# tbennun/capital

Hardware: NVIDIA H100
Metric: cholesky_tflops_fp64 (higher is better)
Workload: dtype f64

## Files before the change

capital_b200/csrc/api.cu:

```cuda
#include "common.cuh"
#include "dist.cuh"
#include "peer.cuh"
#include <math.h>
#include <stdlib.h>
#include <algorithm>

capital_status_t capital_ctx::workspace(const std::string& name, size_t bytes, void** out) {
  capital_ctx* ctx = this;
  DeviceBuf& b = pool[name];
  if (b.bytes < bytes) {
    if (b.p) CAP_CUDA(cudaFree(b.p));
    b.p = nullptr; b.bytes = 0;
    CAP_CUDA(cudaMalloc(&b.p, bytes));
    b.bytes = bytes;
    if (poison_workspace) {
      CAP_CUDA(cudaMemsetAsync(b.p, 0xFF, bytes, cudaStreamLegacy));
      CAP_CUDA(cudaStreamSynchronize(cudaStreamLegacy));
    }
  }
  *out = b.p;
  return CAPITAL_OK;
}

int capital_ctx::stream_id(cudaStream_t st) const {
  if (st == hi) return 1;
  if (st == side) return 2;
  if (st == side_deep[0]) return 3;
  if (st == side_deep[1]) return 4;
  if (peer) {
    const Peer* P = (const Peer*)peer;
    for (int q = 0; q < PEER_Q; q++) if (st == P->push[q]) return 5 + q;
  }
  if (st == copy_in) return 10;
  if (st == copy_out) return 11;
  return 0;
}
int capital_ctx::tl_begin(cudaStream_t st, int kind, double a, double b, double c) {
  if (!timeline) return -1;
  while (tl_pool.size() < tl_used + 2) {
    cudaEvent_t e;
    if (cudaEventCreate(&e) != cudaSuccess) return -1;
    tl_pool.push_back(e);
  }
  TlRec r{tl_pool[tl_used], tl_pool[tl_used + 1], stream_id(st), kind, a, b, c};
  tl_used += 2;
  cudaEventRecord(r.e0, st);
  tl.push_back(r);
  return (int)tl.size() - 1;
}
void capital_ctx::tl_end(cudaStream_t st, int idx) {
  if (idx >= 0) cudaEventRecord(tl[idx].e1, st);
}

bool cap_is_device_ptr(const void* p) {
  cudaPointerAttributes at;
  if (cudaPointerGetAttributes(&at, p) != cudaSuccess) { cudaGetLastError(); return false; }
  return at.type == cudaMemoryTypeDevice || at.type == cudaMemoryTypeManaged;
}

capital_status_t cap_stage_in(capital_ctx* ctx, const double* src, size_t count, const char* name, const double** out) {
  if (cap_is_device_ptr(src)) { *out = src; return CAPITAL_OK; }
  void* d;
  CAP_TRY(ctx->workspace(name, count * 8, &d));
  CAP_CUDA(cudaMemcpyAsync(d, src, count * 8, cudaMemcpyHostToDevice, ctx->stream));
  ctx->counters.h2d_bytes += (int64_t)count * 8;
  *out = (const double*)d;
  return CAPITAL_OK;
}
capital_status_t cap_stage_out_begin(capital_ctx* ctx, double* dst, size_t count, const char* name, double** dev) {
  if (cap_is_device_ptr(dst)) { *dev = dst; return CAPITAL_OK; }
  void* d;
  CAP_TRY(ctx->workspace(name, count * 8, &d));
  *dev = (double*)d;
  return CAPITAL_OK;
}
capital_status_t cap_stage_out_end(capital_ctx* ctx, double* dst, size_t count, const double* dev) {
  if (dev == dst) return CAPITAL_OK;
  CAP_CUDA(cudaMemcpyAsync(dst, dev, count * 8, cudaMemcpyDeviceToHost, ctx->stream));
  ctx->counters.d2h_bytes += (int64_t)count * 8;
  return CAPITAL_OK;
}

capital_status_t cap_check_info(capital_ctx* ctx) {
  int info = 0;
  CAP_CUDA(cudaMemcpyAsync(&info, ctx->d_info, sizeof(int), cudaMemcpyDeviceToHost, ctx->stream));
  CAP_CUDA(cudaStreamSynchronize(ctx->stream));
  if (info == -3) {
    ctx->set_error("the experimental TF32 trailing-update kernel gave up on an mbarrier wait (gemm_tf32.cu watchdog): results are invalid");
    return CAPITAL_ERR_CUDA;
  }
  if (info < 0) {
    ctx->set_error("a wait on a peer GPU timed out (a rank of the grid died, or the ranks did not make the same sequence of calls)");
    return CAPITAL_ERR_COMM;
  }
  if (info != 0) {
    ctx->set_error("matrix is not positive definite: non-positive pivot " + std::to_string(info) + " in a base-case block");
    return CAPITAL_ERR_NOT_SPD;
  }
  return CAPITAL_OK;
}

namespace {
struct HostIO {
  capital_ctx* ctx = nullptr;
  int64_t L = 0, ld = 0;
  double *Rm = nullptr, *Ri = nullptr, *dR = nullptr, *dRinv = nullptr, *hR = nullptr, *hRinv = nullptr;
  bool packed = true;
  std::vector<std::pair<int64_t, cudaEvent_t>> chunks;
  int64_t waited = 0;
  int64_t cols_out = 0, rinv_cols_out = 0;
  bool rinv_streams = false;
  cudaEvent_t e_out = nullptr;
};
capital_status_t io_event(capital_ctx* ctx, cudaEvent_t* e) {
  if (ctx->io_used == ctx->io_pool.size()) {
    cudaEvent_t ev;
    CAP_CUDA(cudaEventCreateWithFlags(&ev, cudaEventDisableTiming));
    ctx->io_pool.push_back(ev);
  }
  *e = ctx->io_pool[ctx->io_used++];
  return CAPITAL_OK;
}
capital_status_t hostio_need_cols(void* user, cudaStream_t st, int64_t col_end) {
  HostIO* io = (HostIO*)user;
  capital_ctx* ctx = io->ctx;
  if (col_end <= io->waited) return CAPITAL_OK;
  for (auto& ch : io->chunks)
    if (ch.first >= col_end) {
      CAP_CUDA(cudaStreamWaitEvent(st, ch.second, 0));
      io->waited = ch.first;
      return CAPITAL_OK;
    }
  return CAPITAL_OK;
}
capital_status_t hostio_left_done(void* user, cudaStream_t st, int64_t col_end, int depth) {
  HostIO* io = (HostIO*)user;
  capital_ctx* ctx = io->ctx;
  const int64_t c0 = io->cols_out;
  if (col_end <= c0) return CAPITAL_OK;
  const bool rinv_too = depth == 0 || (depth == 1 && io->rinv_streams && io->rinv_cols_out == c0);
  const size_t off = (size_t)c0 * (c0 + 1) / 2, cnt = (size_t)col_end * (col_end + 1) / 2 - off;
  cudaStream_t ps = (!ctx->no_overlap && !io->hR && !io->hRinv) ? ctx->copy_out : st;
  cudaEvent_t e;
  if (ps != st) {
    CAP_TRY(io_event(ctx, &e));
    CAP_CUDA(cudaEventRecord(e, st));
    CAP_CUDA(cudaStreamWaitEvent(ps, e, 0));
  }
  CAP_TRY(pack_upper(ctx, ps, io->L, io->Rm, io->ld, io->dR, 0, c0, col_end));
  if (rinv_too) CAP_TRY(pack_upper(ctx, ps, io->L, io->Ri, io->ld, io->dRinv, 0, c0, col_end));
  io->cols_out = col_end;
  if (rinv_too) io->rinv_cols_out = col_end;
  if (!io->hR && !io->hRinv) {
    if (ps != st) {
      CAP_TRY(io_event(ctx, &io->e_out));
      CAP_CUDA(cudaEventRecord(io->e_out, ps));
    }
    return CAPITAL_OK;
  }
  CAP_TRY(io_event(ctx, &e));
  CAP_CUDA(cudaEventRecord(e, ps));
  CAP_CUDA(cudaStreamWaitEvent(ctx->copy_out, e, 0));
  if (io->hR) { CAP_CUDA(cudaMemcpyAsync(io->hR + off, io->dR + off, cnt * 8, cudaMemcpyDeviceToHost, ctx->copy_out)); ctx->counters.d2h_bytes += (int64_t)cnt * 8; }
  if (io->hRinv && rinv_too) { CAP_CUDA(cudaMemcpyAsync(io->hRinv + off, io->dRinv + off, cnt * 8, cudaMemcpyDeviceToHost, ctx->copy_out)); ctx->counters.d2h_bytes += (int64_t)cnt * 8; }
  CAP_TRY(io_event(ctx, &io->e_out));
  CAP_CUDA(cudaEventRecord(io->e_out, ctx->copy_out));
  return CAPITAL_OK;
}
int64_t hostio_cols_waited(void* user) { return ((HostIO*)user)->waited; }
capital_status_t hostio_emit(HostIO* io, cudaStream_t st, bool r_part, int64_t col_end) {
  capital_ctx* ctx = io->ctx;
// ... 458 lines not shown
  const int64_t s1 = L >> args->split;
  const bool packed = structure == CAPITAL_UPPERTRI_PACKED;
  const size_t f_count = packed ? (size_t)L * (L + 1) / 2 : (size_t)L * L;
  const int64_t ldu = packed ? 0 : L;
  cudaStream_t st = ctx->stream;
  const double *dRi = nullptr, *dR = nullptr, *dB;
  if (!apply_r) CAP_TRY(cap_stage_in(ctx, Rinv_local, f_count, "solve_Rinv", &dRi));
  if (skipped || apply_r) CAP_TRY(cap_stage_in(ctx, R_local, f_count, "solve_R", &dR));
  CAP_TRY(cap_stage_in(ctx, B, (size_t)ldb * (nrhs - 1) + n, "solve_B", &dB));
  const bool x_host = !cap_is_device_ptr(X);
  double* dX = X;
  if (x_host) CAP_TRY(ctx->workspace("solve_X", (size_t)ldx * nrhs * 8, (void**)&dX));
  double *T, *T2;
  CAP_TRY(ctx->workspace("solve_T", (size_t)L * SOLVE_W * 8, (void**)&T));
  CAP_TRY(ctx->workspace("solve_T2", (size_t)L * SOLVE_W * 8, (void**)&T2));
  auto half_t = [&](const double* Bp, int64_t w) -> capital_status_t {
    if (!skipped) return tri_apply(ctx, st, {dRi, ldu, true, 0, L, 0, L, w, 1.0, Bp, 1, ldb, 0.0, nullptr, 0, T, 1, L});
    CAP_TRY(tri_apply(ctx, st, {dRi, ldu, true, 0, s1, 0, s1, w, 1.0, Bp, 1, ldb, 0.0, nullptr, 0, T, 1, L}));
    CAP_TRY(tri_apply(ctx, st, {dR, ldu, true, 0, s1, s1, L, w, -1.0, T, 1, L, 1.0, Bp, ldb, T2, 1, L}));
    return tri_apply(ctx, st, {dRi, ldu, true, s1, L, s1, L, w, 1.0, T2, 1, L, 0.0, nullptr, 0, T, 1, L});
  };
  auto half_n = [&](double* Xp, int64_t w) -> capital_status_t {
    if (!skipped) return tri_apply(ctx, st, {dRi, ldu, false, 0, L, 0, L, w, 1.0, T, 1, L, 0.0, nullptr, 0, Xp, 1, ldx});
    CAP_TRY(tri_apply(ctx, st, {dRi, ldu, false, s1, L, s1, L, w, 1.0, T, 1, L, 0.0, nullptr, 0, Xp, 1, ldx}));
    CAP_TRY(tri_apply(ctx, st, {dR, ldu, false, 0, s1, s1, L, w, -1.0, Xp, 1, ldx, 1.0, T, L, T2, 1, L}));
    return tri_apply(ctx, st, {dRi, ldu, false, 0, s1, 0, s1, w, 1.0, T2, 1, L, 0.0, nullptr, 0, Xp, 1, ldx});
  };
  for (int64_t p0 = 0; p0 < nrhs; p0 += SOLVE_W) {
    const int64_t w = std::min<int64_t>(SOLVE_W, nrhs - p0);
    const double* Bp = dB + p0 * ldb;
    double* Xp = dX + p0 * ldx;
    if (apply_r) {
      CAP_TRY(panel_add(ctx, st, L, w, Bp, ldb, nullptr, 0, T, L));
      CAP_TRY(tri_apply(ctx, st, {dR, ldu, mode == SOLVE_RT, 0, L, 0, L, w, 1.0, T, 1, L, 0.0, nullptr, 0, Xp, 1, ldx}));
      continue;
    }
    if (mode != SOLVE_RINV) CAP_TRY(half_t(Bp, w));
    else CAP_TRY(panel_add(ctx, st, L, w, Bp, ldb, nullptr, 0, T, L));
    if (mode != SOLVE_RINVT) CAP_TRY(half_n(Xp, w));
    else CAP_TRY(panel_add(ctx, st, L, w, T, L, nullptr, 0, Xp, ldx));
  }
  if (x_host) {
    CAP_CUDA(cudaMemcpy2DAsync(X, (size_t)ldx * 8, dX, (size_t)ldx * 8, (size_t)n * 8, (size_t)nrhs, cudaMemcpyDeviceToHost, st));
    ctx->counters.d2h_bytes += n * nrhs * 8;
    CAP_CUDA(cudaStreamSynchronize(st));
  }
  return CAPITAL_OK;
}

capital_status_t capital_cholinv_solve_f64(capital_ctx* ctx, int64_t n, const capital_cholinv_args_t* args, capital_structure_t structure,
                                           const double* R_local, const double* Rinv_local, int64_t nrhs, const double* B, int64_t ldb,
                                           double* X, int64_t ldx) {
  if (!ctx) return CAPITAL_ERR_INVALID;
  return cholinv_solve_mode(ctx, n, args, structure, R_local, Rinv_local, nrhs, B, ldb, X, ldx, SOLVE_FULL, "solve");
}

capital_status_t capital_cholinv_apply_rinv_f64(capital_ctx* ctx, int64_t n, const capital_cholinv_args_t* args, capital_structure_t structure,
                                                const double* R_local, const double* Rinv_local, int trans, int64_t nrhs, const double* B,
                                                int64_t ldb, double* X, int64_t ldx) {
  if (!ctx) return CAPITAL_ERR_INVALID;
  if (trans != 0 && trans != 1) {
    ctx->set_error("cholinv::apply_rinv: trans must be 0 (X = R^-1 B) or 1 (X = R^-T B)");
    return CAPITAL_ERR_INVALID;
  }
  return cholinv_solve_mode(ctx, n, args, structure, R_local, Rinv_local, nrhs, B, ldb, X, ldx, trans ? SOLVE_RINVT : SOLVE_RINV,
                            "apply_rinv");
}

capital_status_t capital_cholinv_apply_r_f64(capital_ctx* ctx, int64_t n, const capital_cholinv_args_t* args, capital_structure_t structure,
                                             const double* R_local, int trans, int64_t nrhs, const double* B, int64_t ldb, double* X,
                                             int64_t ldx) {
  if (!ctx) return CAPITAL_ERR_INVALID;
  if (trans != 0 && trans != 1) {
    ctx->set_error("cholinv::apply_r: trans must be 0 (X = R B) or 1 (X = R^T B)");
    return CAPITAL_ERR_INVALID;
  }
  return cholinv_solve_mode(ctx, n, args, structure, R_local, nullptr, nrhs, B, ldb, X, ldx, trans ? SOLVE_RT : SOLVE_R, "apply_r");
}

constexpr size_t BATCHED_WORKSPACE_CAP = size_t(2) << 30;

static int batched_cluster_width(int64_t nb) {
  const char* e = getenv("CAPITAL_BATCHED_CW");
  if (e && atoi(e) == 8) return 8;
  const int64_t T = nb / 64;
  return T <= 2 ? 2 : T <= 4 ? 4 : 8;
}

static bool all_device(std::initializer_list<const void*> ptrs) {
  for (const void* p : ptrs)
    if (!cap_is_device_ptr(p)) return false;
  return true;
}

capital_status_t capital_cholinv_factor_batched_f64(capital_ctx* ctx, int64_t n, int64_t batch, const double* A, double* R, double* Rinv,
                                                    int* info) {
  if (!ctx) return CAPITAL_ERR_INVALID;
  if (!A || !R || !Rinv || !info || n < 1 || batch < 1) {
    ctx->set_error("cholinv::factor_batched: invalid arguments (A, R, Rinv, info non-null, n >= 1, batch >= 1)");
    return CAPITAL_ERR_INVALID;
  }
  if (n > BASECASE_MAX) {
    ctx->set_error("cholinv::factor_batched: n > 512 is not supported (factor each matrix with capital_cholinv_factor_f64)");
    return CAPITAL_ERR_UNSUPPORTED;
  }
  CAP_CUDA(cudaSetDevice(ctx->device));
  if (!all_device({A, R, Rinv, info})) {
    ctx->set_error("cholinv::factor_batched: A, R, Rinv and info must be device pointers");
    return CAPITAL_ERR_INVALID;
  }
  cudaStream_t st = ctx->stream;
  const int64_t nn = n * n;
  CAP_CUDA(cudaMemsetAsync(info, 0, (size_t)batch * sizeof(int), st));
  if (n <= LEAF_MAX) {
    for (int64_t b0 = 0; b0 < batch; b0 += INT32_MAX) {
      const LeafBatch bt{std::min<int64_t>(INT32_MAX, batch - b0), {nn, nn, nn, 0}, info + b0, 0};
      CAP_TRY(leaf_cholinv(ctx, st, (int)n, A + b0 * nn, n, R + b0 * nn, n, Rinv + b0 * nn, n, nullptr, 0, &bt));
    }
    return CAPITAL_OK;
  }
  const int64_t nb = round_up(n, 64), mm = nb * nb;
  const bool direct = nb == n && (((uintptr_t)R | (uintptr_t)Rinv) & 15) == 0;
  const int64_t chunk = std::min<int64_t>({batch, 65535, (int64_t)(BATCHED_WORKSPACE_CAP / ((direct ? 2 : 4) * mm * 8))});
  double *W, *RiT, *Rw = nullptr, *Riw = nullptr;
  CAP_TRY(ctx->workspace("batched_W", (size_t)(chunk * mm) * 8, (void**)&W));
  CAP_TRY(ctx->workspace("batched_RiT", (size_t)(chunk * mm) * 8, (void**)&RiT));
  if (!direct) {
    CAP_TRY(ctx->workspace("batched_R", (size_t)(chunk * mm) * 8, (void**)&Rw));
    CAP_TRY(ctx->workspace("batched_Ri", (size_t)(chunk * mm) * 8, (void**)&Riw));
  }
  const int cw = batched_cluster_width(nb);
  for (int64_t b0 = 0; b0 < batch; b0 += chunk) {
    const int64_t cnt = std::min(chunk, batch - b0);
    CAP_TRY(sym_pad_batched(ctx, st, n, nb, cnt, A + b0 * nn, W));
    if (direct) {
      CAP_CUDA(cudaMemsetAsync(Rinv + b0 * nn, 0, (size_t)(cnt * nn) * 8, st));
      const LeafBatch bt{cnt, {mm, nn, nn, mm}, info + b0, cw};
      CAP_TRY(basecase_cholinv(ctx, st, (int)nb, W, nb, R + b0 * nn, n, Rinv + b0 * nn, n, RiT, nb, &bt));
    } else {
      const LeafBatch bt{cnt, {mm, mm, mm, mm}, info + b0, cw};
      CAP_TRY(basecase_cholinv(ctx, st, (int)nb, W, nb, Rw, nb, Riw, nb, RiT, nb, &bt));
      CAP_TRY(triu_out_batched(ctx, st, n, cnt, Rw, nb, mm, R + b0 * nn));
      CAP_TRY(triu_out_batched(ctx, st, n, cnt, Riw, nb, mm, Rinv + b0 * nn));
    }
  }
  return CAPITAL_OK;
}

capital_status_t capital_cholinv_solve_batched_f64(capital_ctx* ctx, int64_t n, int64_t batch, const double* Rinv, int64_t nrhs,
                                                   const double* B, double* X) {
  if (!ctx) return CAPITAL_ERR_INVALID;
  if (!Rinv || !B || !X || n < 1 || batch < 1 || nrhs < 1) {
    ctx->set_error("cholinv::solve_batched: invalid arguments (Rinv, B, X non-null, n >= 1, batch >= 1, nrhs >= 1)");
    return CAPITAL_ERR_INVALID;
  }
  if (n > BASECASE_MAX) {
    ctx->set_error("cholinv::solve_batched: n > 512 is not supported");
    return CAPITAL_ERR_UNSUPPORTED;
  }
  CAP_CUDA(cudaSetDevice(ctx->device));
  if (!all_device({Rinv, B, X})) {
    ctx->set_error("cholinv::solve_batched: Rinv, B and X must be device pointers");
    return CAPITAL_ERR_INVALID;
  }
  cudaStream_t st = ctx->stream;
  const int64_t nn = n * n, nbk = n * nrhs, ts = n * SOLVE_W;
  const int64_t per = (ts + round_up(n, 64) * SOLVE_W) * 8;
// ... 343 lines not shown
```

capital_b200/csrc/leaf.cu:

```cuda
#include "common.cuh"
#include <cooperative_groups.h>
#include <cfloat>
#include <stdlib.h>
#include <type_traits>
namespace cg = cooperative_groups;

namespace {
constexpr int LD = LEAF_MAX + 1;
constexpr int TLD = 68;
constexpr int TILE_DOUBLES = 64 * TLD;

__device__ __forceinline__ double fast_rsqrt(double d) {
  if (!(d > 1e-30 && d < 1e30)) return rsqrt(d);
  double y = (double)rsqrtf((float)d);
  const double h = 0.5 * d;
  y = y * fma(-h, y * y, 1.5);
  y = y * fma(-h, y * y, 1.5);
  return y;
}

__device__ void leaf_factor_invert(int nb, double* __restrict__ a, double* __restrict__ r, double* __restrict__ t, int* info,
                                   int pivot_base) {
  const int tid = threadIdx.x, tx = tid & 15, ty = tid >> 4;
  for (int k = 0; k < nb; k++) {
    if (tid < 64 && tid >= k && tid < nb) {
      double d = a[k + k * LD];
      if (!(d > 0.0)) {
        if (tid == k) atomicCAS(info, 0, pivot_base + k + 1);
        d = 1.0;
      }
      const double rs = rsqrt(d);
      r[k + tid * LD] = (tid == k) ? d * rs : a[k + tid * LD] * rs;
    }
    __syncthreads();
#pragma unroll
    for (int ia = 0; ia < 4; ia++) {
      const int i = ty + 16 * ia;
      if (i > k && i < nb) {
        const double ri = r[k + i * LD];
#pragma unroll
        for (int jb = 0; jb < 4; jb++) {
          const int j = tx + 16 * jb;
          if (j >= i && j < nb) a[i + j * LD] -= ri * r[k + j * LD];
        }
      }
    }
    __syncthreads();
  }
#pragma unroll
  for (int ia = 0; ia < 4; ia++) {
    const int i = ty + 16 * ia;
#pragma unroll
    for (int jb = 0; jb < 4; jb++) {
      const int j = tx + 16 * jb;
      if (i < nb && j < nb) {
        if (i > j) r[i + j * LD] = 0.0;
        a[i + j * LD] = (i == j) ? 1.0 / r[i + i * LD] : 0.0;
      }
    }
  }
  __syncthreads();
  int lg = 0;
  for (int bs = 1; bs < nb; bs <<= 1, lg++) {
    const int span = 2 * bs;
    const int npairs = (nb + span - 1) / span;
    const int per = bs * bs, total = npairs * per;
    for (int idx = tid; idx < total; idx += 256) {
      const int p = idx >> (2 * lg), e = idx & (per - 1);
      const int li = e & (bs - 1), lj = e >> lg;
      const int o = p * span, i = o + li, j = o + bs + lj;
      if (j < nb) {
        double s = 0.0;
        const int kend = o + bs;
        for (int k = i; k < kend; k++) s += a[i + k * LD] * r[k + j * LD];
        t[i + j * LD] = s;
      }
    }
    __syncthreads();
    for (int idx = tid; idx < total; idx += 256) {
      const int p = idx >> (2 * lg), e = idx & (per - 1);
      const int li = e & (bs - 1), lj = e >> lg;
      const int o = p * span, i = o + li, j = o + bs + lj;
      if (j < nb) {
        double s = 0.0;
        for (int k = o + bs; k <= j; k++) s += t[i + k * LD] * a[k + j * LD];
        a[i + j * LD] = -s;
      }
// ... 233 lines not shown
      sXb[(16 + jl) * TLD + i] = -s;
      sXTb[i * TLD + 16 + jl] = -s;
    });
    (void)tr;
  }
  __syncwarp();
  if (dbg2 && lane == 0) dbg2[2] = clock64();
}

__device__ __forceinline__ void mma32(double (&acc)[2][2], const double* As, int ar, const double* Bs, int bc, int k0) {
  const int lane = threadIdx.x & 31, w = threadIdx.x >> 5, g = lane >> 2, q = lane & 3;
  const double* ap = As + (ar + (w & 3) * 8 + g) * TLD + k0 + q;
  const double* bp = Bs + (bc + (w >> 2) * 16 + g) * TLD + k0 + q;
#pragma unroll
  for (int k = 0; k < 32; k += 4) {
    const double a = ap[k], b0 = bp[k], b1 = bp[8 * TLD + k];
    dmma884(acc[0][0], acc[0][1], a, b0);
    dmma884(acc[1][0], acc[1][1], a, b1);
  }
}
#define M32_ROW ((w & 3) * 8 + g)
#define M32_COL(j, e) ((w >> 2) * 16 + (j) * 8 + 2 * q + (e))

__device__ void leaf64_fast(double* __restrict__ sA, double* __restrict__ sR, double* __restrict__ sX, double* __restrict__ sXT,
                            double* __restrict__ ub, int* info, int pivot_base, long long* dbg2 = nullptr) {
  const int tid = threadIdx.x, lane = tid & 31, w = tid >> 5, g = lane >> 2, q = lane & 3;
  for (int idx = tid; idx < 64 * 64; idx += 256) {
    const int r = idx & 63, cidx = idx >> 6;
    sR[cidx * TLD + r] = 0.0; sX[cidx * TLD + r] = 0.0; sXT[cidx * TLD + r] = 0.0;
  }
  __syncthreads();
  double c[32];
#pragma unroll 1
  for (int half = 0; half < 2; half++) {
    const int o = half * 32;
    if (half == 1) {
      double acc[2][2] = {{0.0, 0.0}, {0.0, 0.0}};
      mma32(acc, sX, 0, sA, 32, 0);
#pragma unroll
      for (int j = 0; j < 2; j++)
#pragma unroll
        for (int e = 0; e < 2; e++) sR[(32 + M32_COL(j, e)) * TLD + M32_ROW] = acc[j][e];
      __syncthreads();
      double acc2[2][2] = {{0.0, 0.0}, {0.0, 0.0}};
      mma32(acc2, sR + 32 * TLD, 0, sR + 32 * TLD, 0, 0);
#pragma unroll
      for (int j = 0; j < 2; j++)
#pragma unroll
        for (int e = 0; e < 2; e++) sA[(32 + M32_COL(j, e)) * TLD + 32 + M32_ROW] -= acc2[j][e];
      __syncthreads();
    }
    if (w == 0) {
#pragma unroll
      for (int i = 0; i < 32; i++) c[i] = sA[(o + lane) * TLD + o + i];
      warp_potrf_trtri_32(c, sR + o * TLD + o, sX + o * TLD + o, sXT + o * TLD + o, ub, lane, info, pivot_base + o,
                          (dbg2 && half == 0) ? dbg2 : nullptr);
      if (dbg2 && half == 0 && lane == 0) dbg2[3] = clock64();
    }
    __syncthreads();
  }
  {
    double acc[2][2] = {{0.0, 0.0}, {0.0, 0.0}};
    mma32(acc, sXT, 0, sR, 32, 0);
    __syncthreads();
#pragma unroll
    for (int j = 0; j < 2; j++)
#pragma unroll
      for (int e = 0; e < 2; e++) sA[M32_ROW * TLD + 32 + M32_COL(j, e)] = acc[j][e];
    __syncthreads();
    double acc2[2][2] = {{0.0, 0.0}, {0.0, 0.0}};
    mma32(acc2, sA, 0, sX, 32, 32);
#pragma unroll
    for (int j = 0; j < 2; j++)
#pragma unroll
      for (int e = 0; e < 2; e++) {
        const double v = -acc2[j][e];
        sX[(32 + M32_COL(j, e)) * TLD + M32_ROW] = v;
        sXT[M32_ROW * TLD + 32 + M32_COL(j, e)] = v;
      }
  }
  __syncthreads();
}

template <int CW>
__global__ void __cluster_dims__(CW, 1, 1) __launch_bounds__(256, 1)
    basecase_kernel(int nb, double* __restrict__ W, long long ldw, double* __restrict__ R, long long ldr, double* __restrict__ Ri,
                    long long ldri, double* __restrict__ RiT, long long ldrit, int* __restrict__ info, long long* __restrict__ dbg,
                    BatchStrides bstr) {
  {
    const long long b = blockIdx.y;
    W += b * bstr.w; R += b * bstr.r; Ri += b * bstr.ri; RiT += b * bstr.rit; info += b;
  }
  extern __shared__ __align__(16) double sm[];
  double* sA = sm;
  double* sB = sm + TILE_DOUBLES;
  double* sT = sm + 2 * TILE_DOUBLES;
  cg::cluster_group cluster = cg::this_cluster();
  const int rank = (int)cluster.block_rank();
  const int T = nb >> 6;
  double acc[4][2][2];
  int dbgi = 0;
#define DBG_STAMP() do { if (dbg && rank == 0 && threadIdx.x == 0) dbg[dbgi++] = clock64(); } while (0)
  DBG_STAMP();

  double* sU = sm + 3 * TILE_DOUBLES;
  auto do_leaf = [&](int jb) {
    const long long o = (long long)jb * 64;
    __syncthreads();
    tile_load(sA, W + o + o * ldw, ldw);
    __syncthreads();
    if (dbg && jb == 0 && threadIdx.x == 0) dbg[20] = clock64();
    leaf64_fast(sA, sB, sT, sU, sm + 4 * TILE_DOUBLES, info, jb * 64, (dbg && jb == 0) ? dbg + 24 : nullptr);
    if (dbg && jb == 0 && threadIdx.x == 0) dbg[21] = clock64();
    tile_store<false>(R + o + o * ldr, ldr, sB);
    tile_store<false>(Ri + o + o * ldri, ldri, sT);
    tile_store<false>(RiT + o + o * ldrit, ldrit, sU);
    __syncthreads();
  };
  auto do_trailing = [&](int jb, int i, int j) {
    const long long o = (long long)jb * 64;
    __syncthreads();
    tile_load(sA, R + o + (long long)i * 64 * ldr, ldr);
    tile_load(sB, R + o + (long long)j * 64 * ldr, ldr);
    __syncthreads();
    acc_zero(acc);
    tile_mma(acc, sA, sB);
    acc_to_smem_colmajor(acc, sT, -1.0);
    __syncthreads();
    tile_store<true>(W + (long long)i * 64 + (long long)j * 64 * ldw, ldw, sT);
  };

  if (rank == 0) do_leaf(0);
  DBG_STAMP();
  __threadfence();
  cluster.sync();
  DBG_STAMP();
  for (int jb = 0; jb < T; jb++) {
    const long long o = (long long)jb * 64;
    int work = 0;
    for (int j = jb + 1; j < T; j++, work++) {
      if (work % CW != rank) continue;
      __syncthreads();
      tile_load(sA, Ri + o + o * ldri, ldri);
      tile_load(sB, W + o + (long long)j * 64 * ldw, ldw);
      __syncthreads();
      acc_zero(acc);
      tile_mma(acc, sA, sB);
      acc_to_smem_colmajor(acc, sT, 1.0);
      __syncthreads();
      tile_store<false>(R + o + (long long)j * 64 * ldr, ldr, sT);
    }
    if (jb == 0) DBG_STAMP();
    __threadfence();
    cluster.sync();
    if (jb == 0) DBG_STAMP();
    if (jb + 1 < T) {
      const int leaf_rank = (jb + 1) % CW;
      if (rank == leaf_rank) {
        do_trailing(jb, jb + 1, jb + 1);
        __threadfence_block();
        do_leaf(jb + 1);
      } else {
        const int slot = rank > leaf_rank ? rank - 1 : rank;
        work = 0;
        for (int j = jb + 1; j < T; j++)
          for (int i = jb + 1; i <= j; i++) {
            if (i == jb + 1 && j == jb + 1) continue;
            if (work++ % (CW - 1) != slot) continue;
            do_trailing(jb, i, j);
          }
      }
    }
    if (jb == 0) DBG_STAMP();
    __threadfence();
    cluster.sync();
    if (jb == 0) DBG_STAMP();
  }
  DBG_STAMP();
  {
    int work = 0;
    for (int j = 0; j < T; j++)
      for (int i = j + 1; i < T; i++, work++) {
        if (work % CW != rank) continue;
        for (int idx = threadIdx.x; idx < 4096; idx += 256)
          R[(long long)i * 64 + (idx & 63) + ((long long)j * 64 + (idx >> 6)) * ldr] = 0.0;
      }
  }
  for (int bs = 1; bs < T; bs <<= 1) {
    const int span = 2 * bs;
    int work = 0;
    for (int o = 0; o + bs < T; o += span) {
      const int jend = min(o + span, T);
      for (int j = o + bs; j < jend; j++)
        for (int i = o; i < o + bs; i++, work++) {
          if (work % CW != rank) continue;
          acc_zero(acc);
          for (int k = i; k < o + bs; k++) {
            __syncthreads();
            tile_load(sA, RiT + (long long)k * 64 + (long long)i * 64 * ldrit, ldrit);
            tile_load(sB, R + (long long)k * 64 + (long long)j * 64 * ldr, ldr);
            __syncthreads();
            tile_mma(acc, sA, sB);
          }
          __syncthreads();
          acc_to_smem_rowmajor(acc, sT, 1.0);
          __syncthreads();
          tile_store_from_rowmajor(W + (long long)j * 64 + (long long)i * 64 * ldw, ldw, sT);
        }
    }
    __threadfence();
    cluster.sync();
    work = 0;
    for (int o = 0; o + bs < T; o += span) {
      const int jend = min(o + span, T);
      for (int j = o + bs; j < jend; j++)
        for (int i = o; i < o + bs; i++, work++) {
          if (work % CW != rank) continue;
          acc_zero(acc);
          for (int k = o + bs; k <= j; k++) {
            __syncthreads();
            tile_load(sA, W + (long long)k * 64 + (long long)i * 64 * ldw, ldw);
            tile_load(sB, Ri + (long long)k * 64 + (long long)j * 64 * ldri, ldri);
            __syncthreads();
            tile_mma(acc, sA, sB);
          }
          __syncthreads();
          acc_to_smem_colmajor(acc, sA, -1.0);
          acc_to_smem_rowmajor(acc, sB, -1.0);
          __syncthreads();
          tile_store<false>(Ri + (long long)i * 64 + (long long)j * 64 * ldri, ldri, sA);
          tile_store_from_rowmajor(RiT + (long long)j * 64 + (long long)i * 64 * ldrit, ldrit, sB);
        }
    }
    __threadfence();
    cluster.sync();
  }
  DBG_STAMP();
}
}

namespace {
constexpr int LEAF_SMEM = 3 * LEAF_MAX * LD * (int)sizeof(double);
constexpr int BASECASE_SMEM = (4 * TILE_DOUBLES + 128 + 512 + 256) * (int)sizeof(double);
}
capital_status_t leaf_init(capital_ctx* ctx) {
  CAP_CUDA(cudaFuncSetAttribute(leaf_kernel, cudaFuncAttributeMaxDynamicSharedMemorySize, LEAF_SMEM));
  CAP_CUDA(cudaFuncSetAttribute(basecase_kernel<2>, cudaFuncAttributeMaxDynamicSharedMemorySize, BASECASE_SMEM));
  CAP_CUDA(cudaFuncSetAttribute(basecase_kernel<4>, cudaFuncAttributeMaxDynamicSharedMemorySize, BASECASE_SMEM));
  CAP_CUDA(cudaFuncSetAttribute(basecase_kernel<8>, cudaFuncAttributeMaxDynamicSharedMemorySize, BASECASE_SMEM));
  return CAPITAL_OK;
}

capital_status_t leaf_cholinv(capital_ctx* ctx, cudaStream_t st, int nb, const double* W, int64_t ldw, double* R, int64_t ldr, double* Ri,
                              int64_t ldri, double* RiT, int64_t ldrit, const LeafBatch* bt) {
  if (nb <= 0) return CAPITAL_OK;
  if (nb > LEAF_MAX || (bt && (bt->batch < 1 || bt->batch > INT32_MAX))) return CAPITAL_ERR_INVALID;
  constexpr int smem = LEAF_SMEM;
  const int tli = ctx->tl_begin(st, 4, nb);
  leaf_kernel<<<bt ? (unsigned)bt->batch : 1u, 256, smem, st>>>(nb, W, ldw, R, ldr, Ri, ldri, RiT, ldrit, bt ? bt->info : ctx->d_info,
                                                                bt ? bt->s : BatchStrides{});
  ctx->tl_end(st, tli);
  ctx->counters.kernel_launches++;
  ctx->counters.leaf_launches++;
  CAP_CUDA(cudaGetLastError());
  return CAPITAL_OK;
}

capital_status_t basecase_cholinv(capital_ctx* ctx, cudaStream_t st, int nb, double* W, int64_t ldw, double* R, int64_t ldr, double* Ri,
                                  int64_t ldri, double* RiT, int64_t ldrit, const LeafBatch* bt) {
  if (nb % 64 != 0 || nb < 64 || nb > BASECASE_MAX || RiT == nullptr) return CAPITAL_ERR_INVALID;
  const int cw = bt ? bt->cw : 8;
  if (bt && (bt->batch < 1 || bt->batch > 65535)) return CAPITAL_ERR_INVALID;
  auto kernel = cw == 2 ? basecase_kernel<2> : cw == 4 ? basecase_kernel<4> : cw == 8 ? basecase_kernel<8> : nullptr;
  if (!kernel) return CAPITAL_ERR_INVALID;
  constexpr int smem = BASECASE_SMEM;
  long long* dbg = nullptr;
  if (getenv("CAPITAL_BC_DEBUG") && !bt) {
    CAP_TRY(ctx->workspace("bc_dbg", 64 * sizeof(long long), (void**)&dbg));
    CAP_CUDA(cudaMemsetAsync(dbg, 0, 64 * sizeof(long long), st));
  }
  const int tli = ctx->tl_begin(st, 3, nb);
  kernel<<<dim3(cw, bt ? (unsigned)bt->batch : 1u), 256, smem, st>>>(nb, W, ldw, R, ldr, Ri, ldri, RiT, ldrit, bt ? bt->info : ctx->d_info,
                                                                      dbg, bt ? bt->s : BatchStrides{});
  ctx->tl_end(st, tli);
  if (dbg) {
    long long h[32];
    CAP_CUDA(cudaMemcpyAsync(h, dbg, sizeof(h), cudaMemcpyDeviceToHost, st));
    CAP_CUDA(cudaStreamSynchronize(st));
    fprintf(stderr, "[bc nb=%d] leaf0=%lld bar=%lld panel0=%lld bar=%lld trail0+leaf1=%lld bar=%lld | chol_total=%lld inverse=%lld total=%lld cycles\n", nb,
            h[1] - h[0], h[2] - h[1], h[3] - h[2], h[4] - h[3], h[5] - h[4], h[6] - h[5], h[7] - h[0], h[8] - h[7], h[8] - h[0]);
    fprintf(stderr, "   leaf64: load=%lld total=%lld | warp32: pre=%lld potrf=%lld trtri=%lld store=%lld\n", h[20] - h[0], h[21] - h[20], h[24] - h[20],
            h[25] - h[24], h[26] - h[25], h[27] - h[26]);
  }
  ctx->counters.kernel_launches++;
  ctx->counters.leaf_launches++;
  CAP_CUDA(cudaGetLastError());
  return CAPITAL_OK;
}
```

Baseline: 32.50.

## Replace cluster barriers in base case with per-tile dataflow flags and critical-path chain

Rewrites the cluster base-case kernel so that, instead of a cluster.sync after every phase, each tile task (panel, trailing update, triangular inverse pieces) waits on release/acquire flags held in the owning block's distributed shared memory and publishes its own flag when done. Rank 0 runs the critical diagonal chain (panel, update, next leaf), while the other ranks take the remaining tasks through a greedy load balancer. Tile loads use cp.async with double buffering. This is meant to remove barrier stalls and let the inverse work overlap the factorization. In exchange it uses more shared memory, adds spin-waits bounded by a 2 s timeout with a new error code, and reworks the debug tracing.

```diff
diff --git a/capital_b200/csrc/api.cu b/capital_b200/csrc/api.cu
--- a/capital_b200/csrc/api.cu
+++ b/capital_b200/csrc/api.cu
@@ -87,6 +87,10 @@
   CAP_CUDA(cudaStreamSynchronize(ctx->stream));
   if (info == -3) {
     ctx->set_error("the experimental TF32 trailing-update kernel gave up on an mbarrier wait (gemm_tf32.cu watchdog): results are invalid");
+    return CAPITAL_ERR_CUDA;
+  }
+  if (info == -4) {
+    ctx->set_error("the cluster base case gave up on a tile wait (leaf.cu, 2 s bound): results are invalid");
     return CAPITAL_ERR_CUDA;
   }
   if (info < 0) {
@@ -711,7 +715,7 @@
 
 static int batched_cluster_width(int64_t nb) {
   const char* e = getenv("CAPITAL_BATCHED_CW");
-  if (e && atoi(e) == 8) return 8;
+  if (e && (atoi(e) == 2 || atoi(e) == 4 || atoi(e) == 8)) return atoi(e);
   const int64_t T = nb / 64;
   return T <= 2 ? 2 : T <= 4 ? 4 : 8;
 }
diff --git a/capital_b200/csrc/leaf.cu b/capital_b200/csrc/leaf.cu
--- a/capital_b200/csrc/leaf.cu
+++ b/capital_b200/csrc/leaf.cu
@@ -3,6 +3,10 @@
 #include <cfloat>
 #include <stdlib.h>
 #include <type_traits>
+#include <algorithm>
+#include <climits>
+#include <string>
+#include <vector>
 namespace cg = cooperative_groups;
 
 namespace {
@@ -402,6 +406,52 @@
   __syncthreads();
 }
 
+constexpr int BC_T = BASECASE_MAX / 64;
+constexpr int SL_LEAF = 0, SL_PANEL = SL_LEAF + BC_T, SL_TRAIL = SL_PANEL + BC_T * BC_T, SL_TINV = SL_TRAIL + BC_T * BC_T * BC_T,
+              SL_RINV = SL_TINV + BC_T * BC_T, BC_NSLOT = SL_RINV + BC_T * BC_T;
+constexpr int BC_WAIT_TIMEOUT = -4;
+constexpr int BC_DBG_TASKS = 64;
+enum { K_LEAF = 0, K_PANEL, K_TRAIL, K_TINV, K_RINV, K_ZERO, K_CHAIN };
+
+__device__ __forceinline__ int sl_panel(int c, int j) { return SL_PANEL + c * BC_T + j; }
+__device__ __forceinline__ int sl_trail(int c, int i, int j) { return SL_TRAIL + (c * BC_T + i) * BC_T + j; }
+__device__ __forceinline__ int sl_tinv(int i, int j) { return SL_TINV + i * BC_T + j; }
+__device__ __forceinline__ int sl_rinv(int i, int j) { return i == j ? SL_LEAF + j : SL_RINV + i * BC_T + j; }
+__device__ __forceinline__ int inv_bs(int i, int j) { return 1 << (31 - __clz(i ^ j)); }
+
+__device__ __forceinline__ unsigned long long gtimer() {
+  unsigned long long t;
+  asm volatile("mov.u64 %0, %%globaltimer;" : "=l"(t));
+  return t;
+}
+__device__ __forceinline__ void flag_set(int* f) {
+  asm volatile("st.release.cluster.u32 [%0], %1;" ::"l"(f), "r"(1) : "memory");
+}
+__device__ __forceinline__ int flag_get(const int* f) {
+  int v;
+  asm volatile("ld.acquire.cluster.u32 %0, [%1];" : "=r"(v) : "l"(f) : "memory");
+  return v;
+}
+__device__ __forceinline__ bool flag_wait(const int* f, const int* info) {
+  if (flag_get(f)) return true;
+  const unsigned long long t0 = gtimer();
+  for (unsigned spin = 1;; spin++) {
+    if (flag_get(f)) return true;
+    if ((spin & 1023u) == 0u && (gtimer() - t0 > 2000000000ull || *(volatile const int*)info == BC_WAIT_TIMEOUT)) return false;
+  }
+}
+__device__ __forceinline__ void tile_load_async(double* dst, const double* src, long long ld) {
+  const int k2 = (threadIdx.x & 31) * 2, c0 = threadIdx.x >> 5;
+#pragma unroll
+  for (int r = 0; r < 8; r++) {
+    const unsigned d = (unsigned)__cvta_generic_to_shared(dst + (c0 + 8 * r) * TLD + k2);
+    asm volatile("cp.async.cg.shared.global [%0], [%1], 16;" ::"r"(d), "l"(src + k2 + (long long)(c0 + 8 * r) * ld) : "memory");
+  }
+  asm volatile("cp.async.commit_group;" ::: "memory");
+}
+template <int N>
+__device__ __forceinline__ void cp_async_wait() { asm volatile("cp.async.wait_group %0;" ::"n"(N) : "memory"); }
+
 template <int CW>
 __global__ void __cluster_dims__(CW, 1, 1) __launch_bounds__(256, 1)
     basecase_kernel(int nb, double* __restrict__ W, long long ldw, double* __restrict__ R, long long ldr, double* __restrict__ Ri,
@@ -415,153 +465,268 @@
   double* sA = sm;
   double* sB = sm + TILE_DOUBLES;
   double* sT = sm + 2 * TILE_DOUBLES;
+  double* sU = sm + 3 * TILE_DOUBLES;
+  double* sE = sm + 4 * TILE_DOUBLES;
+  double* sF = sm + 5 * TILE_DOUBLES;
+  double* ub = sm + 6 * TILE_DOUBLES;
+  int* flags = reinterpret_cast<int*>(ub + 896);
+  unsigned char* owner = reinterpret_cast<unsigned char*>(flags + BC_NSLOT);
+  __shared__ int s_abort;
   cg::cluster_group cluster = cg::this_cluster();
   const int rank = (int)cluster.block_rank();
   const int T = nb >> 6;
-  double acc[4][2][2];
-  int dbgi = 0;
-#define DBG_STAMP() do { if (dbg && rank == 0 && threadIdx.x == 0) dbg[dbgi++] = clock64(); } while (0)
-  DBG_STAMP();
-
-  double* sU = sm + 3 * TILE_DOUBLES;
-  auto do_leaf = [&](int jb) {
-    const long long o = (long long)jb * 64;
-    __syncthreads();
-    tile_load(sA, W + o + o * ldw, ldw);
-    __syncthreads();
-    if (dbg && jb == 0 && threadIdx.x == 0) dbg[20] = clock64();
-    leaf64_fast(sA, sB, sT, sU, sm + 4 * TILE_DOUBLES, info, jb * 64, (dbg && jb == 0) ? dbg + 24 : nullptr);
-    if (dbg && jb == 0 && threadIdx.x == 0) dbg[21] = clock64();
+  const int tid = threadIdx.x;
+  for (int s = tid; s < BC_NSLOT; s += 256) flags[s] = 0;
+  if (tid == 0) s_abort = 0;
+  cluster.sync();
+
+  bool aborted = false;
+  long long* dlog = dbg ? dbg + (long long)rank * BC_DBG_TASKS * 4 : nullptr;
+  int dn = 0;
+  unsigned long long dt0 = 0, dt1 = 0;
+  auto stamp_begin = [&]() { if (dlog && tid == 0) dt0 = gtimer(); };
+  auto stamp_end = [&](int kind, int a, int b, int c) {
+    if (dlog && tid == 0 && dn < BC_DBG_TASKS) {
+      long long* e = dlog + 4 * dn++;
+      e[0] = 1 + kind + 8 * (a + 8 * (b + 8 * c)); e[1] = (long long)dt0; e[2] = (long long)dt1; e[3] = (long long)gtimer();
+    }
+  };
+  auto wait_slot = [&](int slot) {
+    if (tid == 0 && !s_abort && owner[slot] != rank && !flag_wait(cluster.map_shared_rank(flags + slot, (int)owner[slot]), info)) {
+      atomicExch(info, BC_WAIT_TIMEOUT);
+      s_abort = 1;
+    }
+  };
+  auto waits_done = [&]() {
+    __syncthreads();
+    aborted = s_abort != 0;
+    if (dlog && tid == 0) dt1 = gtimer();
+    return !aborted;
+  };
+  auto publish = [&](int slot) {
+    __syncthreads();
+    if (tid == 0) flag_set(flags + slot);
+  };
+
+  auto chain_leaf = [&](int j) {
+    const long long o = (long long)j * 64;
+    leaf64_fast(sE, sB, sT, sU, ub, info, j * 64);
     tile_store<false>(R + o + o * ldr, ldr, sB);
     tile_store<false>(Ri + o + o * ldri, ldri, sT);
     tile_store<false>(RiT + o + o * ldrit, ldrit, sU);
-    __syncthreads();
-  };
-  auto do_trailing = [&](int jb, int i, int j) {
-    const long long o = (long long)jb * 64;
-    __syncthreads();
-    tile_load(sA, R + o + (long long)i * 64 * ldr, ldr);
-    tile_load(sB, R + o + (long long)j * 64 * ldr, ldr);
-    __syncthreads();
+    publish(SL_LEAF + j);
+  };
+  auto chain_step = [&](int c) {
+    const long long o = (long long)c * 64, o1 = o + 64;
+    stamp_begin();
+    if (c > 0) {
+      wait_slot(sl_trail(c - 1, c, c + 1));
+      wait_slot(sl_trail(c - 1, c + 1, c + 1));
+    }
+    if (!waits_done()) return;
+    tile_load_async(sA, W + o + o1 * ldw, ldw);
+    tile_load_async(sE, W + o1 + o1 * ldw, ldw);
+    cp_async_wait<1>();
+    __syncthreads();
+    double acc[4][2][2];
     acc_zero(acc);
-    tile_mma(acc, sA, sB);
+    tile_mma(acc, sT, sA);
+    acc_to_smem_colmajor(acc, sB, 1.0);
+    __syncthreads();
+    tile_store<false>(R + o + o1 * ldr, ldr, sB);
+    acc_zero(acc);
+    tile_mma(acc, sB, sB);
+    cp_async_wait<0>();
+    publish(sl_panel(c, c + 1));
+    {
+      const int lane = tid & 31, w = tid >> 5, g = lane >> 2, q = lane & 3;
+#pragma unroll
+      for (int i = 0; i < 4; i++)
+#pragma unroll
+        for (int jj = 0; jj < 2; jj++)
+#pragma unroll
+          for (int e = 0; e < 2; e++) {
+            double& x = sE[TILE_COL(jj, e) * TLD + TILE_ROW(i)];
+            x = -1.0 * acc[i][jj][e] + x;
+          }
+    }
+    __syncthreads();
+    chain_leaf(c + 1);
+    stamp_end(K_CHAIN, c, 0, 0);
+  };
+
+  auto chain_last_rinv = [&](int i, int j) {
+    stamp_begin();
+    wait_slot(sl_tinv(i, j));
+    if (!waits_done()) return;
+    tile_load(sA, W + (long long)j * 64 + (long long)i * 64 * ldw, ldw);
+    __syncthreads();
+    double acc[4][2][2];
+    acc_zero(acc);
+    tile_mma(acc, sA, sT);
+    acc_to_smem_colmajor(acc, sB, -1.0);
+    acc_to_smem_rowmajor(acc, sU, -1.0);
+    __syncthreads();
+    tile_store<false>(Ri + (long long)i * 64 + (long long)j * 64 * ldri, ldri, sB);
+    tile_store_from_rowmajor(RiT + (long long)j * 64 + (long long)i * 64 * ldrit, ldrit, sU);
+    publish(sl_rinv(i, j));
+    stamp_end(K_RINV, i, j, 0);
+  };
+
+  auto kloop = [&](double (&acc)[4][2][2], int k0, int k1, auto srcA, auto srcB) {
+    acc_zero(acc);
+    tile_load_async(sA, srcA(k0).p, srcA(k0).ld);
+    tile_load_async(sB, srcB(k0).p, srcB(k0).ld);
+    for (int k = k0; k <= k1; k++) {
+      double* a = ((k - k0) & 1) ? sE : sA;
+      double* b = ((k - k0) & 1) ? sF : sB;
+      if (k < k1) {
+        tile_load_async(((k - k0) & 1) ? sA : sE, srcA(k + 1).p, srcA(k + 1).ld);
+        tile_load_async(((k - k0) & 1) ? sB : sF, srcB(k + 1).p, srcB(k + 1).ld);
+        cp_async_wait<2>();
+      } else {
+        cp_async_wait<0>();
+      }
+      __syncthreads();
+      tile_mma(acc, a, b);
+      __syncthreads();
+    }
+  };
+  struct Src { const double* p; long long ld; };
+  auto do_panel = [&](int c, int j) {
+    const long long o = (long long)c * 64;
+    stamp_begin();
+    wait_slot(SL_LEAF + c);
+    if (c > 0) wait_slot(sl_trail(c - 1, c, j));
+    if (!waits_done()) return;
+    double acc[4][2][2];
+    kloop(acc, c, c, [&](int) { return Src{Ri + o + o * ldri, ldri}; },
+          [&](int) { return Src{W + o + (long long)j * 64 * ldw, ldw}; });
+    acc_to_smem_colmajor(acc, sT, 1.0);
+    __syncthreads();
+    tile_store<false>(R + o + (long long)j * 64 * ldr, ldr, sT);
+    publish(sl_panel(c, j));
+    stamp_end(K_PANEL, c, j, 0);
+  };
+  auto do_trail = [&](int c, int i, int j) {
+    const long long o = (long long)c * 64;
+    stamp_begin();
+    wait_slot(sl_panel(c, i));
+    wait_slot(sl_panel(c, j));
+    if (c > 0) wait_slot(sl_trail(c - 1, i, j));
+    if (!waits_done()) return;
+    double acc[4][2][2];
+    kloop(acc, c, c, [&](int) { return Src{R + o + (long long)i * 64 * ldr, ldr}; },
+          [&](int) { return Src{R + o + (long long)j * 64 * ldr, ldr}; });
     acc_to_smem_colmajor(acc, sT, -1.0);
     __syncthreads();
     tile_store<true>(W + (long long)i * 64 + (long long)j * 64 * ldw, ldw, sT);
-  };
-
-  if (rank == 0) do_leaf(0);
-  DBG_STAMP();
-  __threadfence();
+    publish(sl_trail(c, i, j));
+    stamp_end(K_TRAIL, c, i, j);
+  };
+  auto do_tinv = [&](int i, int j) {
+    const int bs = inv_bs(i, j), kend = (i & ~(2 * bs - 1)) + bs - 1;
+    stamp_begin();
+    for (int k = i; k <= kend; k++) { wait_slot(sl_rinv(i, k)); wait_slot(sl_panel(k, j)); }
+    if (!waits_done()) return;
+    double acc[4][2][2];
+    kloop(acc, i, kend, [&](int k) { return Src{RiT + (long long)k * 64 + (long long)i * 64 * ldrit, ldrit}; },
+          [&](int k) { return Src{R + (long long)k * 64 + (long long)j * 64 * ldr, ldr}; });
+    acc_to_smem_rowmajor(acc, sT, 1.0);
+    __syncthreads();
+    tile_store_from_rowmajor(W + (long long)j * 64 + (long long)i * 64 * ldw, ldw, sT);
+    publish(sl_tinv(i, j));
+    stamp_end(K_TINV, i, j, 0);
+  };
+  auto do_rinv = [&](int i, int j) {
+    const int bs = inv_bs(i, j), kbeg = (i & ~(2 * bs - 1)) + bs;
+    stamp_begin();
+    for (int k = kbeg; k <= j; k++) { wait_slot(sl_tinv(i, k)); wait_slot(sl_rinv(k, j)); }
+    if (!waits_done()) return;
+    double acc[4][2][2];
+    kloop(acc, kbeg, j, [&](int k) { return Src{W + (long long)k * 64 + (long long)i * 64 * ldw, ldw}; },
+          [&](int k) { return Src{Ri + (long long)k * 64 + (long long)j * 64 * ldri, ldri}; });
+    acc_to_smem_colmajor(acc, sT, -1.0);
+    acc_to_smem_rowmajor(acc, sU, -1.0);
+    __syncthreads();
+    tile_store<false>(Ri + (long long)i * 64 + (long long)j * 64 * ldri, ldri, sT);
+    tile_store_from_rowmajor(RiT + (long long)j * 64 + (long long)i * 64 * ldrit, ldrit, sU);
+    publish(sl_rinv(i, j));
+    stamp_end(K_RINV, i, j, 0);
+  };
+  auto do_zero = [&](int i, int j) {
+    for (int idx = tid; idx < 4096; idx += 256)
+      R[(long long)i * 64 + (idx & 63) + ((long long)j * 64 + (idx >> 6)) * ldr] = 0.0;
+  };
+
+  int load[CW > 1 ? CW - 1 : 1];
+#pragma unroll
+  for (int w = 0; w < CW - 1; w++) load[w] = 0;
+  auto take = [&](int slot, int cost) {
+    int best = 0, bl = load[0];
+#pragma unroll
+    for (int w = 1; w < CW - 1; w++)
+      if (load[w] < bl) { bl = load[w]; best = w; }
+#pragma unroll
+    for (int w = 0; w < CW - 1; w++) load[w] += (w == best) ? cost : 0;
+    if (tid == 0 && slot >= 0) owner[slot] = (unsigned char)(best + 1);
+    return !aborted && rank == best + 1;
+  };
+  auto chain_owns = [&](int slot) { if (tid == 0) owner[slot] = 0; };
+
+  chain_owns(SL_LEAF + 0);
+  if (rank == 0) {
+    stamp_begin();
+    tile_load(sE, W, ldw);
+    if (dlog && tid == 0) dt1 = gtimer();
+    __syncthreads();
+    chain_leaf(0);
+    stamp_end(K_LEAF, 0, 0, 0);
+  }
+  for (int j = 0; j < T; j++)
+    for (int i = j + 1; i < T; i++)
+      if (take(-1, 1)) do_zero(i, j);
+  for (int c = 0; c + 1 < T; c++) {
+    chain_owns(sl_panel(c, c + 1));
+    chain_owns(sl_trail(c, c + 1, c + 1));
+    chain_owns(SL_LEAF + c + 1);
+    if (rank == 0 && !aborted) chain_step(c);
+    for (int j = c + 2; j < T; j++)
+      if (take(sl_panel(c, j), 1)) do_panel(c, j);
+    if (c + 2 < T) {
+      if (take(sl_trail(c, c + 1, c + 2), 1)) do_trail(c, c + 1, c + 2);
+      if (take(sl_trail(c, c + 2, c + 2), 1)) do_trail(c, c + 2, c + 2);
+    }
+    for (int i = c + 1; i < T; i++)
+      for (int j = i; j < T; j++) {
+        if ((i == c + 1 && j <= c + 2) || (i == c + 2 && j == c + 2)) continue;
+        if (take(sl_trail(c, i, j), 1)) do_trail(c, i, j);
+      }
+    const int j = c + 1;
+    for (int i = 0; i < j; i++) {
+      const int bs = inv_bs(i, j), kend = (i & ~(2 * bs - 1)) + bs - 1;
+      if (take(sl_tinv(i, j), kend - i + 1)) do_tinv(i, j);
+    }
+    for (int bs = 1; bs < T; bs <<= 1) {
+      if (!(j & bs)) continue;
+      const int o = j & ~(2 * bs - 1);
+      for (int i = o; i < o + bs; i++) {
+        if (bs == 1 && j == T - 1) {
+          chain_owns(sl_rinv(i, j));
+          if (rank == 0 && !aborted) chain_last_rinv(i, j);
+        } else if (take(sl_rinv(i, j), j - (o + bs) + 1)) {
+          do_rinv(i, j);
+        }
+      }
+    }
+  }
   cluster.sync();
-  DBG_STAMP();
-  for (int jb = 0; jb < T; jb++) {
-    const long long o = (long long)jb * 64;
-    int work = 0;
-    for (int j = jb + 1; j < T; j++, work++) {
-      if (work % CW != rank) continue;
-      __syncthreads();
-      tile_load(sA, Ri + o + o * ldri, ldri);
-      tile_load(sB, W + o + (long long)j * 64 * ldw, ldw);
-      __syncthreads();
-      acc_zero(acc);
-      tile_mma(acc, sA, sB);
-      acc_to_smem_colmajor(acc, sT, 1.0);
-      __syncthreads();
-      tile_store<false>(R + o + (long long)j * 64 * ldr, ldr, sT);
-    }
-    if (jb == 0) DBG_STAMP();
-    __threadfence();
-    cluster.sync();
-    if (jb == 0) DBG_STAMP();
-    if (jb + 1 < T) {
-      const int leaf_rank = (jb + 1) % CW;
-      if (rank == leaf_rank) {
-        do_trailing(jb, jb + 1, jb + 1);
-        __threadfence_block();
-        do_leaf(jb + 1);
-      } else {
-        const int slot = rank > leaf_rank ? rank - 1 : rank;
-        work = 0;
-        for (int j = jb + 1; j < T; j++)
-          for (int i = jb + 1; i <= j; i++) {
-            if (i == jb + 1 && j == jb + 1) continue;
-            if (work++ % (CW - 1) != slot) continue;
-            do_trailing(jb, i, j);
-          }
-      }
-    }
-    if (jb == 0) DBG_STAMP();
-    __threadfence();
-    cluster.sync();
-    if (jb == 0) DBG_STAMP();
-  }
-  DBG_STAMP();
-  {
-    int work = 0;
-    for (int j = 0; j < T; j++)
-      for (int i = j + 1; i < T; i++, work++) {
-        if (work % CW != rank) continue;
-        for (int idx = threadIdx.x; idx < 4096; idx += 256)
-          R[(long long)i * 64 + (idx & 63) + ((long long)j * 64 + (idx >> 6)) * ldr] = 0.0;
-      }
-  }
-  for (int bs = 1; bs < T; bs <<= 1) {
-    const int span = 2 * bs;
-    int work = 0;
-    for (int o = 0; o + bs < T; o += span) {
-      const int jend = min(o + span, T);
-      for (int j = o + bs; j < jend; j++)
-        for (int i = o; i < o + bs; i++, work++) {
-          if (work % CW != rank) continue;
-          acc_zero(acc);
-          for (int k = i; k < o + bs; k++) {
-            __syncthreads();
-            tile_load(sA, RiT + (long long)k * 64 + (long long)i * 64 * ldrit, ldrit);
-            tile_load(sB, R + (long long)k * 64 + (long long)j * 64 * ldr, ldr);
-            __syncthreads();
-            tile_mma(acc, sA, sB);
-          }
-          __syncthreads();
-          acc_to_smem_rowmajor(acc, sT, 1.0);
-          __syncthreads();
-          tile_store_from_rowmajor(W + (long long)j * 64 + (long long)i * 64 * ldw, ldw, sT);
-        }
-    }
-    __threadfence();
-    cluster.sync();
-    work = 0;
-    for (int o = 0; o + bs < T; o += span) {
-      const int jend = min(o + span, T);
-      for (int j = o + bs; j < jend; j++)
-        for (int i = o; i < o + bs; i++, work++) {
-          if (work % CW != rank) continue;
-          acc_zero(acc);
-          for (int k = o + bs; k <= j; k++) {
-            __syncthreads();
-            tile_load(sA, W + (long long)k * 64 + (long long)i * 64 * ldw, ldw);
-            tile_load(sB, Ri + (long long)k * 64 + (long long)j * 64 * ldri, ldri);
-            __syncthreads();
-            tile_mma(acc, sA, sB);
-          }
-          __syncthreads();
-          acc_to_smem_colmajor(acc, sA, -1.0);
-          acc_to_smem_rowmajor(acc, sB, -1.0);
-          __syncthreads();
-          tile_store<false>(Ri + (long long)i * 64 + (long long)j * 64 * ldri, ldri, sA);
-          tile_store_from_rowmajor(RiT + (long long)j * 64 + (long long)i * 64 * ldrit, ldrit, sB);
-        }
-    }
-    __threadfence();
-    cluster.sync();
-  }
-  DBG_STAMP();
 }
 }
 
 namespace {
 constexpr int LEAF_SMEM = 3 * LEAF_MAX * LD * (int)sizeof(double);
-constexpr int BASECASE_SMEM = (4 * TILE_DOUBLES + 128 + 512 + 256) * (int)sizeof(double);
+constexpr int BASECASE_SMEM = (6 * TILE_DOUBLES + 128 + 512 + 256) * (int)sizeof(double) + BC_NSLOT * ((int)sizeof(int) + 1);
 }
 capital_status_t leaf_init(capital_ctx* ctx) {
   CAP_CUDA(cudaFuncSetAttribute(leaf_kernel, cudaFuncAttributeMaxDynamicSharedMemorySize, LEAF_SMEM));
@@ -594,23 +759,41 @@
   auto kernel = cw == 2 ? basecase_kernel<2> : cw == 4 ? basecase_kernel<4> : cw == 8 ? basecase_kernel<8> : nullptr;
   if (!kernel) return CAPITAL_ERR_INVALID;
   constexpr int smem = BASECASE_SMEM;
+  constexpr int DBG_N = 8 * BC_DBG_TASKS * 4;
   long long* dbg = nullptr;
   if (getenv("CAPITAL_BC_DEBUG") && !bt) {
-    CAP_TRY(ctx->workspace("bc_dbg", 64 * sizeof(long long), (void**)&dbg));
-    CAP_CUDA(cudaMemsetAsync(dbg, 0, 64 * sizeof(long long), st));
+    CAP_TRY(ctx->workspace("bc_dbg", DBG_N * sizeof(long long), (void**)&dbg));
+    CAP_CUDA(cudaMemsetAsync(dbg, 0, DBG_N * sizeof(long long), st));
   }
   const int tli = ctx->tl_begin(st, 3, nb);
   kernel<<<dim3(cw, bt ? (unsigned)bt->batch : 1u), 256, smem, st>>>(nb, W, ldw, R, ldr, Ri, ldri, RiT, ldrit, bt ? bt->info : ctx->d_info,
                                                                       dbg, bt ? bt->s : BatchStrides{});
   ctx->tl_end(st, tli);
   if (dbg) {
-    long long h[32];
-    CAP_CUDA(cudaMemcpyAsync(h, dbg, sizeof(h), cudaMemcpyDeviceToHost, st));
+    std::vector<long long> h(DBG_N);
+    CAP_CUDA(cudaMemcpyAsync(h.data(), dbg, DBG_N * sizeof(long long), cudaMemcpyDeviceToHost, st));
     CAP_CUDA(cudaStreamSynchronize(st));
-    fprintf(stderr, "[bc nb=%d] leaf0=%lld bar=%lld panel0=%lld bar=%lld trail0+leaf1=%lld bar=%lld | chol_total=%lld inverse=%lld total=%lld cycles\n", nb,
-            h[1] - h[0], h[2] - h[1], h[3] - h[2], h[4] - h[3], h[5] - h[4], h[6] - h[5], h[7] - h[0], h[8] - h[7], h[8] - h[0]);
-    fprintf(stderr, "   leaf64: load=%lld total=%lld | warp32: pre=%lld potrf=%lld trtri=%lld store=%lld\n", h[20] - h[0], h[21] - h[20], h[24] - h[20],
-            h[25] - h[24], h[26] - h[25], h[27] - h[26]);
+    long long t0 = LLONG_MAX, t1 = 0, last_leaf = 0;
+    for (int i = 0; i < DBG_N; i += 4)
+      if (h[i]) { t0 = std::min(t0, h[i + 1]); t1 = std::max(t1, h[i + 3]); if ((h[i] - 1) % 8 == K_CHAIN || (h[i] - 1) % 8 == K_LEAF) last_leaf = std::max(last_leaf, h[i + 3]); }
+    const char* names[] = {"leaf", "panel", "trail", "tinv", "rinv", "zero", "chain"};
+    fprintf(stderr, "[bc nb=%d] span %.1f us, after the last leaf %.1f us (ns of %%globaltimer from the first task's start)\n", nb,
+            (t1 - t0) * 1e-3, (t1 - last_leaf) * 1e-3);
+    for (int r = 0; r < cw; r++) {
+      long long busy = 0, wait = 0;
+      std::string line;
+      for (int e = 0; e < BC_DBG_TASKS; e++) {
+        const long long* x = h.data() + (r * BC_DBG_TASKS + e) * 4;
+        if (!x[0]) break;
+        const long long tag = x[0] - 1;
+        busy += x[3] - x[2]; wait += x[2] - x[1];
+        char buf[96];
+        snprintf(buf, sizeof(buf), " %s(%lld,%lld,%lld)[w%.1f r%.1f @%.1f]", names[tag % 8], tag / 8 % 8, tag / 64 % 8, tag / 512 % 8,
+                 (x[2] - x[1]) * 1e-3, (x[3] - x[2]) * 1e-3, (x[3] - t0) * 1e-3);
+        line += buf;
+      }
+      fprintf(stderr, "  rank %d: run %.1f us, wait %.1f us:%s\n", r, busy * 1e-3, wait * 1e-3, line.c_str());
+    }
   }
   ctx->counters.kernel_launches++;
   ctx->counters.leaf_launches++;
```

Result: no change. 32.63 (median of 6 runs) (+0.4%).
